# grayhong/self-diagnosing-gan

Hardware: AMD Instinct MI355X
Metric: images/sec (G+D step) (higher is better)
Workload: dtype f32

## Files before the change

### self-diagnosing-gan_amd/csrc/conv_wgrad.hip

```cpp
#include "conv_common.h"
#include "switches.h"
#include <stdlib.h>
#include <type_traits>


namespace diagan {
bool wgrad_wino_supported(int Hi, int Wi, int Ci, int Ho, int Wo, int Co, int R, int S, int sy, int dr, int off, int up,
                          int Kp);
int wgrad_wino_splits(int B, int Ho, int Wo, int Ci, int Co);
int launch_wgrad_wino(WgradArgs a, int splits, int segments, hipStream_t st);
int launch_wgrad_wino_batched(const WgradArgs* jobs, const int* splits, const int* segments, int n, hipStream_t st);
int wgrad_wino_batch_max();
bool wgrad_x3_takes(const WgradArgs& a, bool x3_on);
int launch_wgrad_x3(const WgradArgs& a, int splits, hipStream_t st);
void wgrad_x3_set(int on);


template <int BNn, int BNk, int PRO, bool P2>
__device__ __forceinline__ void conv_wgrad_body(const WgradArgs& a, const int bid, const int nblk) {
  constexpr int BK = 32;
  constexpr int TM = BNn / 64, TN = BNk / 64;
  constexpr int AC = BNn / 4, BC = BNk / 4;
  constexpr int AJ = BK * AC / 256, BJ = BK * BC / 256;
  constexpr int APR = 256 / AC, BPR = 256 / BC;
// ... 356 lines not shown
        for (int u = 0; u < U; ++u)
          t[u][r] = __builtin_bit_cast(f32x4, __builtin_amdgcn_raw_buffer_load_b128(src, voff[u] + (unsigned)r * sbytes, 0, 0));
#pragma unroll
      for (int u = 0; u < U; ++u) {
#pragma unroll
        for (int w = 1; w < R; w <<= 1)
#pragma unroll
          for (int r = 0; r + w < R; r += 2 * w) t[u][r] += t[u][r + w];
        acc[u] += t[u][0];
      }
    }
    if (sn) {
      double dot = 0.0;
      const __amdgpu_buffer_rsrc_t wsrc = __builtin_amdgcn_make_buffer_rsrc(const_cast<float*>(L.W), 0, L.n_w * 4, 0x00020000);
      const __amdgpu_buffer_rsrc_t dst = __builtin_amdgcn_make_buffer_rsrc(sl, 0, L.n_elem * 4, 0x00020000);
      f32x4 wv[U];
#pragma unroll
      for (int u = 0; u < U; ++u) wv[u] = __builtin_bit_cast(f32x4, __builtin_amdgcn_raw_buffer_load_b128(wsrc, voff[u], 0, 0));
#pragma unroll
      for (int u = 0; u < U; ++u) {
        const f32x4 g = acc[u];
        if (L.splits > 1)
          __builtin_amdgcn_raw_buffer_store_b128(__builtin_bit_cast(u32x4_t, g), dst, voff[u], 0, 0);
        dot += (double)g[0] * wv[u][0] + (double)g[1] * wv[u][1] + (double)g[2] * wv[u][2] + (double)g[3] * wv[u][3];
        acc[u] = z4;
      }
      dot = wave_sum(dot);
      __syncthreads();
      if ((threadIdx.x & 63) == 0) red[threadIdx.x >> 6] = dot;
      __syncthreads();
      if (threadIdx.x == 0) L.partials[c][lb] = (red[0] + red[1]) + (red[2] + red[3]);
    }
  }
  if (!sn) {
    const __amdgpu_buffer_rsrc_t gsrc = __builtin_amdgcn_make_buffer_rsrc(L.grad, 0, L.n_elem * 4, 0x00020000);
    f32x4 og[U];
#pragma unroll
    for (int u = 0; u < U; ++u) og[u] = __builtin_bit_cast(f32x4, __builtin_amdgcn_raw_buffer_load_b128(gsrc, voff[u], 0, 0));
#pragma unroll
    for (int u = 0; u < U; ++u)
      __builtin_amdgcn_raw_buffer_store_b128(__builtin_bit_cast(u32x4_t, og[u] + acc[u]), gsrc, voff[u], 0, 0);
  }
}

template <typename F>
__device__ __forceinline__ void fin_dispatch(int U, F&& f) {
  switch (U) {
    case 8: f(std::integral_constant<int, 8>{}); break;
    case 4: f(std::integral_constant<int, 4>{}); break;
    case 2: f(std::integral_constant<int, 2>{}); break;
    default: f(std::integral_constant<int, 1>{}); break;
  }
}

__global__ __launch_bounds__(256) __attribute__((amdgpu_waves_per_eu(4, 4))) void wgrad_finish_a_kernel(const WgFinish* __restrict__ tab, int n_layers) {
  const WgFinish L = load_uniform(tab + find_layer(tab, n_layers, blockIdx.x));
  const int lb = blockIdx.x - L.first_block;
  const int U = fin_u(L.splits);
  if ((long)lb * 1024 * U >= L.n_elem) return;
  __shared__ double red[4];
  fin_dispatch(U, [&](auto u) { fin_a<decltype(u)::value>(L, lb, red); });
}

__global__ __launch_bounds__(256) void wgrad_finish_dot_kernel(const WgFinish* __restrict__ tab) {
  const WgFinish L = tab[blockIdx.x];
  if (L.W == nullptr) return;
  __shared__ double red[256];
  const int fe = 1024 * fin_u(L.splits), nparts = (L.n_elem + fe - 1) / fe;
  for (int c = 0; c < L.nctx; ++c) {
    double d = 0.0;
    for (int k = threadIdx.x; k < nparts; k += 256) d += L.partials[c][k];
    red[threadIdx.x] = d;
    __syncthreads();
    for (int w = 128; w > 0; w >>= 1) {
      if ((int)threadIdx.x < w) red[threadIdx.x] += red[threadIdx.x + w];
      __syncthreads();
    }
    if (threadIdx.x == 0) L.partials[c][nparts] = red[0];
    __syncthreads();
  }
}

template <int U>
__device__ __forceinline__ void fin_b(const WgFinish& L, int lb) {
  constexpr int ELEMS = 1024 * U;
  constexpr int UC = U > 1 ? 2 : 1;
  const int nparts = (L.n_elem + ELEMS - 1) / ELEMS;
  float inv[2] = {0.f, 0.f}, coef[2] = {0.f, 0.f};
#pragma unroll
  for (int c = 0; c < 2; ++c) {
    if (c >= L.nctx) break;
    inv[c] = L.state[c][1];
    coef[c] = (float)(L.partials[c][nparts] * (double)inv[c]);
  }
  const int Co = L.n_w / L.Kp;
  const __amdgpu_buffer_rsrc_t gsrc = __builtin_amdgcn_make_buffer_rsrc(L.grad, 0, L.n_elem * 4, 0x00020000);
  __amdgpu_buffer_rsrc_t qsrc[2], vsrc[2], usrc[2];
#pragma unroll
  for (int c = 0; c < 2; ++c) {
    const bool on = c < L.nctx;
    qsrc[c] = __builtin_amdgcn_make_buffer_rsrc(L.slab[c], 0, on ? L.n_elem * 4 : 0, 0x00020000);
    vsrc[c] = __builtin_amdgcn_make_buffer_rsrc(const_cast<float*>(L.v[c]), 0, on ? L.Kp * 4 : 0, 0x00020000);
    usrc[c] = __builtin_amdgcn_make_buffer_rsrc(const_cast<float*>(L.u[c]), 0, on ? Co * 4 : 0, 0x00020000);
  }
#pragma unroll
  for (int u0 = 0; u0 < U; u0 += UC) {
    unsigned po[UC];
    bool okw[UC];
    f32x4 og[UC], gq[UC][2], vv[UC][2];
    float uu[UC][2];
#pragma unroll
    for (int i = 0; i < UC; ++i) {
      const long pos = (long)lb * ELEMS + ((u0 + i) * 256 + threadIdx.x) * 4;
      po[i] = pos < L.n_elem ? (unsigned)pos * 4u : 0x80000000u;
      okw[i] = pos < L.n_w;
      const unsigned n = okw[i] ? (unsigned)pos / (unsigned)L.Kp : 0u;
      const unsigned ko = okw[i] ? ((unsigned)pos - n * (unsigned)L.Kp) * 4u : 0x80000000u;
      const unsigned no = okw[i] ? n * 4u : 0x80000000u;
      og[i] = __builtin_bit_cast(f32x4, __builtin_amdgcn_raw_buffer_load_b128(gsrc, po[i], 0, 0));
#pragma unroll
      for (int c = 0; c < 2; ++c) {
        gq[i][c] = __builtin_bit_cast(f32x4, __builtin_amdgcn_raw_buffer_load_b128(qsrc[c], po[i], 0, 0));
        vv[i][c] = __builtin_bit_cast(f32x4, __builtin_amdgcn_raw_buffer_load_b128(vsrc[c], ko, 0, 0));
        uu[i][c] = __builtin_bit_cast(float, __builtin_amdgcn_raw_buffer_load_b32(usrc[c], no, 0, 0));
      }
    }
#pragma unroll
    for (int i = 0; i < UC; ++i) {
      f32x4 o = og[i];
#pragma unroll
      for (int c = 0; c < 2; ++c) {
        const f32x4 w = (gq[i][c] - (uu[i][c] * coef[c]) * vv[i][c]) * inv[c];
        o += okw[i] ? w : gq[i][c];
      }
      __builtin_amdgcn_raw_buffer_store_b128(__builtin_bit_cast(u32x4_t, o),
                                             gsrc, po[i], 0, 0);
    }
    __builtin_amdgcn_sched_barrier(0);
  }
}

__global__ __launch_bounds__(256) void wgrad_finish_b_kernel(const WgFinish* __restrict__ tab, int n_layers) {
  const WgFinish L = load_uniform(tab + find_layer(tab, n_layers, blockIdx.x));
  const int lb = blockIdx.x - L.first_block;
  const int U = fin_u(L.splits);
  if (L.W == nullptr || (long)lb * 1024 * U >= L.n_elem) return;
  fin_dispatch(U, [&](auto u) { fin_b<decltype(u)::value>(L, lb); });
}

extern "C" __attribute__((visibility("default"))) int diagan_wgrad_finish_block_elems(int splits) { return 1024 * fin_u(splits); }

}

using namespace diagan;
extern "C" int diagan_conv_gemm_get_wino(void);
extern "C" int diagan_conv_gemm_get_x3b(void);
extern "C" int diagan_conv_wgrad_splits(int M, int Co, int Kp);
extern "C" int diagan_conv_wgrad_uses_wino(int Hi, int Wi, int Ci, int Ho, int Wo, int Co, int R, int S, int sy, int dr,
                                           int off, int up, int Kp);

DIAGAN_API int diagan_wgrad_finish_batched(const void* table_dev, int n_layers, int64_t total_blocks, int any_sn,
                                           void* stream) {
  DG_REQUIRE(table_dev && n_layers > 0 && total_blocks > 0 && total_blocks < (1L << 31), "wgrad_finish_batched: bad args");
  static_assert(sizeof(WgFinish) == 128, "descriptor layout");
  const WgFinish* tab = (const WgFinish*)table_dev;
  hipStream_t st = (hipStream_t)stream;
  hipLaunchKernelGGL(wgrad_finish_a_kernel, dim3((unsigned)total_blocks), dim3(256), 0, st, tab, n_layers);
  if (any_sn) {
    hipLaunchKernelGGL(wgrad_finish_dot_kernel, dim3(n_layers), dim3(256), 0, st, tab);
    hipLaunchKernelGGL(wgrad_finish_b_kernel, dim3((unsigned)total_blocks), dim3(256), 0, st, tab, n_layers);
  }
  return check_launch("wgrad_finish_batched");
}

static void wgrad_tile(int Co, int Kp, int* bn, int* bk) {
  *bn = Co <= 64 ? 64 : 128;
  *bk = Kp <= 64 ? 64 : 128;
  if (*bn == 128 && *bk == 64) *bn = 64;
}

static void wgrad_gemm_fields(WgradArgs& a, int* bn, int* bk, bool* p2) {
  const ConvGeom& g = a.g;
  wgrad_tile(g.Co, g.Kp, bn, bk);
  a.tiles = cdiv(g.Co, *bn) * cdiv(g.Kp, *bk);
  a.same = (g.Hi == g.Ho && g.Wi == g.Wo && g.sy == 1 && g.up == 1) ? 1 : 0;
  *p2 = (g.Ho & (g.Ho - 1)) == 0 && (g.Wo & (g.Wo - 1)) == 0;
  a.lgW = a.lgHW = 0;
  while ((1 << a.lgW) < g.Wo) ++a.lgW;
  while ((1 << a.lgHW) < g.Ho * g.Wo) ++a.lgHW;
}

static int wgrad_fill_args(WgradArgs& a, const float* dy, const float* x, float* slab, int splits, int segments,
                           int64_t slab_stride, int64_t bias_off, const float* pro_scale, const float* pro_shift, int pro_mode, int B,
                           int Hi, int Wi, int Ci, int Ho, int Wo, int Co, int R, int S, int sy, int dr, int off, int up, int Kp) {
  DG_REQUIRE(dy && x && slab, "conv_wgrad: null tensor");
  DG_REQUIRE(B > 0 && Hi > 0 && Wi > 0 && Ho > 0 && Wo > 0 && R > 0 && S > 0, "conv_wgrad: bad dims");
  DG_REQUIRE(Ci > 0 && (Ci & 3) == 0 && Co > 0 && (Co & 3) == 0, "conv_wgrad: Ci=%d, Co=%d must be multiples of 4", Ci, Co);
  DG_REQUIRE(up == 1 || up == 2, "conv_wgrad: up=%d unsupported", up);
  DG_REQUIRE(dr == 1 || dr == -1, "conv_wgrad: dr must be +-1");
  DG_REQUIRE(Kp % 32 == 0 && Kp >= R * S * Ci, "conv_wgrad: bad Kp=%d", Kp);
  DG_REQUIRE(splits >= 1, "conv_wgrad: splits=%d", splits);
  DG_REQUIRE(pro_mode >= 0 && pro_mode <= PRO_BOX_RELU, "conv_wgrad: bad pro_mode %d", pro_mode);
  DG_REQUIRE(!(pro_mode == PRO_BOX || pro_mode == PRO_BOX_RELU) || (up == 1 && dr == 1 && Hi >= 2 && Wi >= 2),
             "conv_wgrad: the box-sum loader (pro_mode 5 / 6) gathers forward geometries without up-sampling");
  DG_REQUIRE(!(pro_mode == PRO_AFFINE_RELU || pro_mode == PRO_AFFINE) || (pro_scale && pro_shift),
             "conv_wgrad: affine prologue needs scale/shift");
  DG_REQUIRE(slab_stride >= (int64_t)Co * Kp && (bias_off < 0 || bias_off + Co <= slab_stride),
             "conv_wgrad: slab_stride=%ld too small for Co*Kp=%ld (+bias)", (long)slab_stride, (long)Co * Kp);
  DG_REQUIRE((long)Co * Kp * 4 < (1L << 31), "conv_wgrad: weight tensor must be smaller than 2 GiB");
  DG_REQUIRE((long)B * Ho * Wo * Co * 4 < (1L << 31) && (long)B * Hi * Wi * Ci * 4 < (1L << 31),
             "conv_wgrad: tensors must be smaller than 2 GiB (32-bit buffer offsets)");
  a.dy = dy; a.x = x; a.slab = slab; a.pro_scale = pro_scale; a.pro_shift = pro_shift; a.pro_mode = pro_mode;
  a.M = B * Ho * Wo;
  a.g = ConvGeom{B, Hi, Wi, Ci, Ho, Wo, Co, R, S, sy, dr, off, up, R * S * Ci, Kp};
  a.dWo = make_fastdiv((unsigned)Wo);
  a.dHo = make_fastdiv((unsigned)Ho);
  a.adv_b = 32 / (Ho * Wo);
  a.adv_y = (32 % (Ho * Wo)) / Wo;
  a.adv_x = (32 % (Ho * Wo)) % Wo;
  const int total_steps = cdiv(a.M, 32);
  DG_REQUIRE(segments >= 1 && splits % segments == 0, "conv_wgrad: splits=%d not a multiple of segments=%d", splits, segments);
  DG_REQUIRE(segments == 1 || (a.M % (32 * segments)) == 0, "conv_wgrad: %d pixels do not split into %d segments of whole K-steps", a.M, segments);
  a.seg_steps = cdiv(total_steps, segments);
  a.splits_per_seg = splits / segments;
  a.steps_per_split = cdiv(a.seg_steps, a.splits_per_seg);
  a.slab_stride = slab_stride;
  a.bias_off = bias_off;
  return DIAGAN_OK;
}

DIAGAN_API int diagan_conv_wgrad(const float* dy, const float* x, float* slab, int splits, int segments,
                                 int64_t slab_stride, int64_t bias_off, const float* pro_scale, const float* pro_shift, int pro_mode, int B,
                                 int Hi, int Wi, int Ci, int Ho, int Wo, int Co, int R, int S, int sy,
                                 int dr, int off, int up, int Kp, void* stream) {
  WgradArgs a;
  const int rc = wgrad_fill_args(a, dy, x, slab, splits, segments, slab_stride, bias_off, pro_scale, pro_shift, pro_mode, B, Hi, Wi, Ci,
                                 Ho, Wo, Co, R, S, sy, dr, off, up, Kp);
  if (rc != DIAGAN_OK) return rc;
  hipStream_t st = (hipStream_t)stream;
  if (diagan_conv_wgrad_uses_wino(Hi, Wi, Ci, Ho, Wo, Co, R, S, sy, dr, off, up, Kp))
    return launch_wgrad_wino(a, splits, segments, st);
  int bn, bk;
  bool p2;
  wgrad_gemm_fields(a, &bn, &bk, &p2);
  if (bn == 128 && bk == 128 && wgrad_x3_takes(a, diagan_conv_gemm_get_x3b() != 0)) return launch_wgrad_x3(a, splits, st);
  const dim3 grid(a.tiles * splits);
#define DG_WG(BN_, PRO_) do { if (p2) hipLaunchKernelGGL((conv_wgrad_kernel<BN_, 128, PRO_, true>), grid, dim3(256), 0, st, a); \
                              else hipLaunchKernelGGL((conv_wgrad_kernel<BN_, 128, PRO_, false>), grid, dim3(256), 0, st, a); } while (0)
#define DG_WG_ALL(BN_) switch (pro_mode) { \
      case PRO_NONE: DG_WG(BN_, PRO_NONE); break; \
      case PRO_RELU: DG_WG(BN_, PRO_RELU); break; \
// ... 156 lines not shown
```

### self-diagnosing-gan_amd/csrc/weight_prep.hip

```cpp
#include "conv_common.h"

namespace diagan {

__global__ __launch_bounds__(256) void sn_gemv_cols_kernel(const float* __restrict__ W, const float* __restrict__ u,
                                                           float* __restrict__ v_raw, int Co, int Kp) {
  const int k = blockIdx.x * 256 + threadIdx.x;
  if (k >= Kp) return;
  float s = 0.f;
  for (int n = 0; n < Co; ++n) s = fmaf(u[n], W[(long)n * Kp + k], s);
  v_raw[k] = s;
}

__global__ __launch_bounds__(256) void sn_gemv_rows_kernel(const float* __restrict__ W, const float* __restrict__ v_raw,
                                                           float* __restrict__ t_raw, int Co, int Kp) {
  const int n = blockIdx.x * 4 + (threadIdx.x >> 6);
  if (n >= Co) return;
  const int lane = threadIdx.x & 63;
  float s = 0.f;
  for (int k = lane * 4; k < Kp; k += 256) {
    const f32x4 w = *reinterpret_cast<const f32x4*>(W + (long)n * Kp + k);
    const f32x4 v = *reinterpret_cast<const f32x4*>(v_raw + k);
    s += w[0] * v[0] + w[1] * v[1] + w[2] * v[2] + w[3] * v[3];
  }
  s = wave_sum(s);
// ... 335 lines not shown
  }
  const float sigma = block_sum_256(s, red);
  if (threadIdx.x == 0) {
    L.state[0] = sigma;
    L.state[1] = 1.f / sigma;
    if (update_buffers) L.sigma_buf[0] = sigma;
  }
}

constexpr int PACK_MAX_LAYERS = 64;
constexpr int PACK_GRID = 2048;
__global__ __launch_bounds__(256) void pack_batched_kernel(const SnLayer* __restrict__ tab, int n_layers, int write_wd) {
  __shared__ float tile[32][33];
  __shared__ int first[PACK_MAX_LAYERS + 1];
  if (threadIdx.x == 0) {
    int acc = 0;
    for (int l = 0; l < n_layers; ++l) {
      first[l] = acc;
      const bool live = tab[l].Wf || (tab[l].Wd && write_wd);
      acc += live ? tab[l].RS * ((tab[l].Ci + 31) / 32) * ((tab[l].Co + 31) / 32) : 0;
    }
    first[n_layers] = acc;
  }
  __syncthreads();
  const int total = first[n_layers];
  const int tx = threadIdx.x & 31, ty = threadIdx.x >> 5;
  int l = 0;
  for (int item = blockIdx.x; item < total; item += gridDim.x) {
    while (first[l + 1] <= item) ++l;
    const SnLayer L = tab[l];
    const int tc = (L.Ci + 31) / 32, tn = (L.Co + 31) / 32;
    int r = item - first[l];
    const int tap = r / (tc * tn);
    r -= tap * (tc * tn);
    const int co0 = (r / tc) * 32, ci0 = (r % tc) * 32;
    const float inv = L.state[1];
    for (int q = ty; q < 32; q += 8) {
      const int co = co0 + q, ci = ci0 + tx;
      float v = 0.f;
      if (co < L.Co && ci < L.Ci) {
        v = L.W[(long)co * L.Kp + tap * L.Ci + ci] * inv;
        if (L.Wf) L.Wf[(long)co * L.Kp + tap * L.Ci + ci] = v;
      }
      tile[q][tx] = v;
    }
    __syncthreads();
    if (L.Wd && write_wd) {
      for (int q = ty; q < 32; q += 8) {
        const int ci = ci0 + q, co = co0 + tx;
        if (ci < L.Ci && co < L.Co) L.Wd[(long)ci * L.Kd + tap * L.Co + co] = tile[tx][q];
      }
    }
    __syncthreads();
  }
}

}

DIAGAN_API int diagan_sn_prepare_batched(const void* table_dev, int n_layers, int max_Co, int max_Ci, int max_RS,
                                         int max_Kp, float eps, int update_buffers, int write_wd, void* stream) {
  DG_REQUIRE(table_dev && n_layers > 0 && max_Co > 0 && max_Ci > 0 && max_RS > 0 && max_Kp > 0,
             "sn_prepare_batched: bad args");
  DG_REQUIRE(max_Kp <= SN_MAX_KP, "sn_prepare_batched: Kp=%d exceeds the LDS-resident limit %d", max_Kp, SN_MAX_KP);
  DG_REQUIRE(n_layers <= PACK_MAX_LAYERS, "sn_prepare_batched: at most %d layers per table", PACK_MAX_LAYERS);
  static_assert(sizeof(SnLayer) == 96, "descriptor layout");
  hipStream_t st = (hipStream_t)stream;
  const SnLayer* tab = (const SnLayer*)table_dev;
  hipLaunchKernelGGL(sn_cols_batched_kernel, dim3(cdiv(max_Kp, 64), SN_RSPLIT, n_layers), dim3(256), 0, st, tab);
  hipLaunchKernelGGL(sn_rows_batched_kernel, dim3(cdiv(max_Co, 8), 1, n_layers), dim3(256), 0, st, tab);
  hipLaunchKernelGGL(sn_finalize_batched_kernel, dim3(1, 1, n_layers), dim3(256), 0, st, tab, eps, update_buffers);
  if (write_wd >= 0)
    hipLaunchKernelGGL(pack_batched_kernel, dim3(PACK_GRID), dim3(256), 0, st, tab, n_layers, write_wd);
  return check_launch("sn_prepare_batched");
}

DIAGAN_API int diagan_pack_batched(const void* table_dev, int n_layers, int max_Co, int max_Ci, int max_RS,
                                   int write_wd, void* stream) {
  DG_REQUIRE(table_dev && n_layers > 0 && max_Co > 0 && max_Ci > 0 && max_RS > 0, "pack_batched: bad args");
  DG_REQUIRE(n_layers <= PACK_MAX_LAYERS, "pack_batched: at most %d layers per table", PACK_MAX_LAYERS);
  hipLaunchKernelGGL(pack_batched_kernel, dim3(PACK_GRID), dim3(256), 0, (hipStream_t)stream, (const SnLayer*)table_dev,
                     n_layers, write_wd);
  return check_launch("pack_batched");
}
```

### self-diagnosing-gan_amd/diagan/models/layers.py

```python

import os

import torch
import torch.nn as nn

from diagan.ops import conv as C
from diagan.ops import eltwise as E

WGRAD_BOX = os.environ.get("DIAGAN_WGRAD_BOX", "1") != "0"


def _r4(n):
    return (n + 3) // 4 * 4


class ConvLayer(nn.Module):

    def __init__(self, kind, in_ch, out_ch, ksize, stride=1, pad=0, bias=True, sn=False, xavier_gain=None):
        super().__init__()
        self.kind, self.in_ch, self.out_ch, self.ksize = kind, in_ch, out_ch, ksize
        self.Cip, self.Cop = _r4(in_ch), _r4(out_ch)
        self.geom = C.Geom(kind, self.Cip, self.Cop, ksize, ksize, stride, pad)
        self.sn = sn
        ref = (nn.Conv2d if kind == 'conv' else nn.ConvTranspose2d)(in_ch, out_ch, ksize, stride, pad, bias=bias)
        self._oihw_shape = tuple(ref.weight.shape)
        self.weight = nn.Parameter(self._pack(ref.weight.data))
        if bias:
            b = torch.zeros(self.Cop)
            b[:out_ch] = ref.bias.data
            self.bias = nn.Parameter(b)
        else:
            self.bias = None
        if sn:
            self.register_buffer('sn_u', torch.randn(1, out_ch))
            self.register_buffer('sn_sigma', torch.ones(1))
        self._wd = None
        self._wd_version = -1
        self._register_state_dict_hook(self._sd_hook)
        self._register_load_state_dict_pre_hook(self._load_hook)
        if xavier_gain is not None:
            self.xavier_(xavier_gain)

    def xavier_(self, gain):
        w = torch.empty(self._oihw_shape)
        nn.init.xavier_uniform_(w, gain)
        self.weight.data.copy_(self._pack(w).to(self.weight.device))
        return self

    def _pack(self, w):
        if self.kind == 'convT':
            w = w.permute(1, 0, 2, 3)
        Co, Ci, R, S = w.shape
        wp = w.permute(0, 2, 3, 1)
        wp = torch.nn.functional.pad(wp, (0, self.Cip - Ci))
        out = torch.zeros((self.Cop, self.geom.Kp), dtype=w.dtype, device=w.device)
        out[:Co, : R * S * self.Cip] = wp.reshape(Co, -1)
        return out

    def _unpack(self, wp):
        R = self.ksize
        w = wp[: self.out_ch, : R * R * self.Cip].reshape(self.out_ch, R, R, self.Cip)[..., : self.in_ch]
        w = w.permute(0, 3, 1, 2)
        if self.kind == 'convT':
            w = w.permute(1, 0, 2, 3)
        return w.contiguous()

    @staticmethod
    def _sd_hook(module, sd, prefix, local_metadata):
        sd[prefix + 'weight'] = module._unpack(sd[prefix + 'weight'])
        if module.bias is not None:
            sd[prefix + 'bias'] = sd[prefix + 'bias'][: module.out_ch].clone()
        return sd

    def _load_hook(self, sd, prefix, *args):
        k = prefix + 'weight'
        if k in sd and sd[k].dim() == 4:
            sd[k] = self._pack(sd[k].to(torch.float32))
        k = prefix + 'bias'
        if k in sd and sd[k].numel() == self.out_ch and self.out_ch != self.Cop:
            b = torch.zeros(self.Cop, dtype=torch.float32, device=sd[k].device)
            b[: self.out_ch] = sd[k]
            sd[k] = b
        net = getattr(self, '_net', None)
        if net is not None:
            net.param_version += 1

    class Ctx:
        __slots__ = ("wf", "wd", "u", "v", "state", "_keep", "row_scale", "pair", "wkey", "wver")

        def __init__(self):
            self.row_scale = None
            self.pair = None
# ... 322 lines not shown
            p0, p1 = ctx.pair
            gx, _, _ = E.head_bwd(dlogit, self.weight.data, p0.state[1:], ctx.x, ctx.pooled, need_gx=True,
                                  need_wgrad=False, inv_sigma1=p1.state[1:])
            if need_wgrad:
                h = dlogit.numel() // 2
                for p, sl in ((p0, slice(0, h)), (p1, slice(h, 2 * h))):
                    _, G, dot = E.head_bwd(dlogit[sl], self.weight.data, None, ctx.x[sl], ctx.pooled[sl], need_gx=False,
                                           need_wgrad=True, dbias=self.bias.grad)
                    nat.call("diagan_sn_grad_fix", nat.ptr(G), nat.ptr(dot), 1, nat.ptr(p.u), nat.ptr(p.v),
                             nat.ptr(p.state), nat.ptr(self.weight.grad), 1, self.in_ch, 1, nat.current_stream())
            return gx
        inv = ctx.state[1:] if self.sn else None
        gx, G, dot = E.head_bwd(dlogit, self.weight.data, inv, ctx.x, ctx.pooled, need_gx=True,
                                need_wgrad=need_wgrad, dbias=self.bias.grad if need_wgrad else None)
        if need_wgrad:
            if self.sn:
                from diagan import _native as nat
                nat.call("diagan_sn_grad_fix", nat.ptr(G), nat.ptr(dot), 1, nat.ptr(ctx.u), nat.ptr(ctx.v),
                         nat.ptr(ctx.state), nat.ptr(self.weight.grad), 1, self.in_ch, 1, nat.current_stream())
            else:
                E.add(self.weight.grad.view(-1), G, out=self.weight.grad.view(-1))
        return gx


class SNBatch:

    def __init__(self, net, layers, n_slots=2):
        import numpy as np
        from diagan import _native as nat
        self.net, self.layers, self.nat = net, layers, nat
        dev = net.flat_params.device
        self.slab_generation = net.slab_generation
        desc = np.dtype([('p', np.uint64, 9), ('i', np.int32, 6)])
        self.tables = []
        f32 = dict(dtype=torch.float32, device=dev)
        dims = []
        for slot in range(n_slots):
            tab = np.zeros(len(layers), dtype=desc)
            for li, m in enumerate(layers):
                if isinstance(m, ConvLayer):
                    g = m.geom
                    Co, Ci, RS, Kp, Kd = g.Co, g.Ci, g.R * g.S, g.Kp, g.Kd
                    wf, wd = torch.zeros((Co, Kp), **f32), torch.zeros((Ci, Kd), **f32)
                    ctx = ConvLayer.Ctx()
                else:
                    Co, Ci, RS, Kp, Kd = 1, m.in_ch, 1, m.in_ch, 0
                    wf = wd = None
                    ctx = HeadLinear.Ctx()
                ctx.u, ctx.v, ctx.state = torch.zeros(Co, **f32), torch.zeros(Kp, **f32), torch.ones(2, **f32)
                if isinstance(m, ConvLayer):
                    ctx.wf, ctx.wd, ctx.wkey = wf, wd, slot
                work = torch.zeros(8 * Kp + Co, **f32)
                ctx._keep = (work,)
                if not hasattr(m, '_slot_ctx') or m._slot_ctx is None or len(m._slot_ctx) != n_slots:
                    m._slot_ctx = [None] * n_slots
                m._slot_ctx[slot] = ctx
                ptrs = [m.weight.data.data_ptr(), m.sn_u.data_ptr(), m.sn_sigma.data_ptr(), ctx.u.data_ptr(),
                        ctx.v.data_ptr(), ctx.state.data_ptr(), work.data_ptr(),
                        wf.data_ptr() if wf is not None else 0, wd.data_ptr() if wd is not None else 0]
                tab[li]['p'] = ptrs
                tab[li]['i'] = [Co, Ci, RS, Kp, Kd, 0]
                dims.append((Co, Ci, RS, Kp))
            self.tables.append(torch.from_numpy(tab.view(np.uint8).copy()).to(dev))
        self.max = [max(d[k] for d in dims) for k in range(4)]
        convs = [m for m in layers if isinstance(m, ConvLayer)]
        self.unit = torch.ones(2, **f32)
        ptab = np.zeros(len(convs), dtype=desc)
        for li, m in enumerate(convs):
            g = m.geom
            wd_raw = torch.zeros((g.Ci, g.Kd), **f32)
            pc = ConvLayer.Ctx()
            pc.wf, pc.wd = m.weight.data, wd_raw
            pc.u = pc.v = pc.state = None
            pc.row_scale = (m._slot_ctx[0].state[1:], m._slot_ctx[1].state[1:])
            pc.pair = (m._slot_ctx[0], m._slot_ctx[1])
            pc.wkey = 'pair'
            m._pair_ctx = pc
            ptab[li]['p'] = [m.weight.data.data_ptr(), 0, 0, 0, 0, self.unit.data_ptr(), 0, 0, wd_raw.data_ptr()]
            ptab[li]['i'] = [g.Co, g.Ci, g.R * g.S, g.Kp, g.Kd, 0]
        self.pair_table = torch.from_numpy(ptab.view(np.uint8).copy()).to(dev)
        self.n_convs = len(convs)
        self.pair_version = None
        self.convs = convs
        self.runs = 0
        self.slot_ver = {}

    def stale(self):
        self.net.flat_params
        return self.slab_generation != self.net.slab_generation

    def run_pair(self, training, need_dgrad):
        self.run(0, training, -1)
        self.run(1, training, -1)
        if need_dgrad and self.pair_version != self.net.param_version:
            nat = self.nat
            nat.call("diagan_pack_batched", self.pair_table.data_ptr(), self.n_convs, self.max[0], self.max[1],
                     self.max[2], 1, nat.current_stream())
            self.pair_version = self.net.param_version
        for m in self.convs:
            m._pair_ctx.wver = ('p', self.net.param_version)

    def run(self, slot, training, write_wd):
        nat = self.nat
        nat.call("diagan_sn_prepare_batched", self.tables[slot].data_ptr(), len(self.layers), self.max[0],
                 self.max[1], self.max[2], self.max[3], 1e-12, 1 if training else 0,
                 write_wd if isinstance(write_wd, int) and not isinstance(write_wd, bool) else (1 if write_wd else 0),
                 nat.current_stream())
        if write_wd != -1:
            self.runs += 1
            self.slot_ver[slot] = ('s', self.runs)
            for m in self.convs:
                m._slot_ctx[slot].wver = self.slot_ver[slot]


class WgradEntry:
    __slots__ = ("owner", "slot", "M", "n_w", "n_elem", "stride", "splits", "own_splits", "bias_off", "segments", "slab",
                 "partials", "sn_ctx")

    def __init__(self, owner, slot, M, n_w, stride, splits, bias_off, segments, dev):
        self.owner, self.slot, self.M, self.n_w, self.n_elem, self.stride = owner, slot, M, n_w, stride, stride
        self.splits, self.own_splits, self.bias_off, self.segments, self.sn_ctx = splits, splits, bias_off, segments, None
        self.slab = torch.empty(splits * stride, dtype=torch.float32, device=dev)
        self.partials = torch.empty((segments, (stride + 1023) // 1024 + 1), dtype=torch.float64, device=dev)

    def set_splits(self, splits):
        if splits != self.splits:
            self.splits = splits
            self.slab = torch.empty(splits * self.stride, dtype=torch.float32, device=self.slab.device)
            self.owner.drop_tables(self.slot)


class WgradBatch:
    QUEUE_BYTES = int(os.environ.get("DIAGAN_WGRAD_QUEUE_BYTES", str(8 << 30)))

    def __init__(self, net):
        self.net = net
        self.entries = {}
        self.launched = {}
        self.tables = {}
        self.slab_generation = None
        self.hold = False
        self.pending = []
        self.overlapped = 0
        self.queue = {}
        self.queued_bytes = {}
        self.batch_plans = {}
        self.job_tables = {}
        self.batched_launches = 0

    def drop_tables(self, slot):
        self.tables = {k: v for k, v in self.tables.items() if k[0] != slot}

    def _entry(self, layer, slot, M, segments, dy_shape, x_shape, geom):
        self.net.flat_grads
        if self.slab_generation != self.net.slab_generation:
            self.entries.clear(), self.tables.clear(), self.job_tables.clear()
            self.slab_generation = self.net.slab_generation
        e = self.entries.get((layer, slot))
        if e is None or e.M != M:
            g = geom if geom is not None else layer.geom
            n_w = g.Co * g.Kp
            has_bias = layer.bias is not None
            n_b = layer.bias.numel() if has_bias else 0
            if has_bias and layer.bias.grad.data_ptr() != layer.weight.grad.data_ptr() + 4 * n_w:
                raise RuntimeError("bias gradient does not follow the weight gradient in the flat slab")
            stride = n_w + n_b
            base = C.wgrad_splits_geom(g, dy_shape[0], x_shape[1], x_shape[2], dy_shape[1], dy_shape[2])
            splits = max(segments, base // segments * segments)
            if segments == 1 and C.small_co_wgrad(g):
                splits = C.small_co_wgrad_splits(dy_shape[0], dy_shape[1])
            e = self.entries[(layer, slot)] = WgradEntry(self, slot, M, n_w, stride, splits, n_w if has_bias else -1, segments,
                                                         layer.weight.device)
            self.drop_tables(slot)
        return e

    def launch(self, layer, slot, dy, x, pro, sn_ctx, segments=1, geom=None):
        M = dy.numel() // dy.shape[-1]
        if self.hold and slot in self.pending:
            self.pending.remove(slot)
            self.flush(slot)
            self._finish_layers(slot, self.launched.pop(slot, []))
        xs = C.wg_x_shape(x, pro)
        e = self._entry(layer, slot, M, segments, tuple(dy.shape), xs, geom)
        e.sn_ctx = sn_ctx
        self.launched.setdefault(slot, []).append(layer)
        g, pooled = (geom, True) if geom is not None else (layer.geom, False)
        if C.WGRAD_BATCH and dy.dim() == 4 and x.dim() == 4:
            mode = int(pro[0]) if pro is not None else 0
            if not (segments == 1 and C.small_co_wgrad(g)) and C.wgrad_batch_class(g, xs[1], xs[2], dy.shape[1], dy.shape[2], mode):
                shape = C.WgradShape(g, tuple(dy.shape), tuple(xs), mode, segments, e.own_splits, pooled)
                self.queue.setdefault(slot, []).append(C.WgradJob(layer, dy, x, pro, e, shape))
                self.queued_bytes[slot] = self.queued_bytes.get(slot, 0) + 4 * (dy.numel() + x.numel())
                if self.queued_bytes[slot] > self.QUEUE_BYTES:
                    self.flush(slot)
                return
        C.conv_wgrad_into(g, dy, x, e.slab, e.splits, e.stride, e.bias_off, pro=pro, segments=segments, pooled=pooled)

    def flush(self, slot):
        jobs = self.queue.pop(slot, None)
        self.queued_bytes.pop(slot, None)
        if not jobs:
            return
        key = tuple(j.shape for j in jobs)
        plan = self.batch_plans.get(key)
        if plan is None:
            plan = self.batch_plans[key] = C.wgrad_launch_plan(key)
        for n, launch in enumerate(plan):
            part = [jobs[j] for j in launch.jobs]
            for job, splits in zip(part, launch.splits):
                job.entry.set_splits(splits)
            if len(part) > 1:
                C.conv_wgrad_batched(part, launch.kernel_name, flop_scale=4.0 if launch.pooled else 1.0, key=(key, n),
                                     cache=self.job_tables)
                self.batched_launches += 1
            else:
                job, e = part[0], part[0].entry
                C.conv_wgrad_into(job.shape.geom, job.dy, job.x, e.slab, e.splits, e.stride, e.bias_off, pro=job.pro,
                                  segments=job.shape.segments, pooled=launch.pooled)

    def finish(self, slot):
        self.flush(slot)
        if self.hold:
            self.pending.append(slot)
            return
        self._finish_layers(slot, self.launched.pop(slot, []))

    def split_for_overlap(self, slot):
        layers = self.launched.get(slot, [])
        if len(layers) < 2:
            return None
        base = self.net.flat_grads.data_ptr()
        lo = [(l.weight.grad.data_ptr() - base) // 4 for l in layers]
        hi = [o + self.entries[(l, slot)].n_elem for o, l in zip(lo, layers)]
        total, acc, best = sum(b - a for a, b in zip(lo, hi)), 0, None
        for h in range(1, len(layers)):
            acc += hi[h - 1] - lo[h - 1]
            cut = min(lo[:h])
            if cut % 4 == 0 and all(b <= cut for b in hi[h:]):
                score = abs(2 * acc - total)
                if best is None or score < best[0]:
                    best = (score, h, cut)
        if best is None:
            return None
        _, h, cut = best
        return layers[:h], layers[h:], cut

    def _finish_layers(self, slot, layers):
        import numpy as np
        from diagan import _native as nat
        if not layers:
            return
        key = (slot, tuple(id(l) for l in layers))
        t = self.tables.get(key)
        if t is None:
            desc = np.dtype([('p', np.uint64, 12), ('stride', np.int64), ('i', np.int32, 6)])
            tab = np.zeros(len(layers), dtype=desc)
            any_sn, total_blocks = 0, 0
            for li, layer in enumerate(layers):
                e = self.entries[(layer, slot)]
                c = e.sn_ctx
                ctxs = list(c) if isinstance(c, tuple) else [c]
                nctx = len(ctxs)
                per = e.splits // nctx
                sn = ctxs[0] is not None
                any_sn |= int(sn)
                pp = [0] * 12
                for pi, cc in enumerate(ctxs):
                    pp[0 + pi] = e.slab.data_ptr() + 4 * pi * per * e.stride
                    if sn:
                        pp[2 + pi], pp[4 + pi], pp[6 + pi] = cc.u.data_ptr(), cc.v.data_ptr(), cc.state.data_ptr()
                    pp[8 + pi] = e.partials[pi].data_ptr()
                if not sn and nctx > 1:
                    nctx, per = 1, e.splits
                pp[10] = layer.weight.grad.data_ptr()
                pp[11] = layer.weight.data.data_ptr() if sn else 0
                assert 64 * e.stride < 2 ** 31, "wgrad finish: 16 splits of a layer must fit a 2 GiB buffer window"
                tab[li]['p'], tab[li]['stride'] = pp, e.stride
                tab[li]['i'] = [per, e.n_elem, e.n_w, layer.geom.Kp, nctx, total_blocks]
                be = nat.fn("diagan_wgrad_finish_block_elems")(per)
                total_blocks += (e.n_elem + be - 1) // be
            t = (torch.from_numpy(tab.view(np.uint8).copy()).to(layers[0].weight.device), len(layers), total_blocks, any_sn)
            self.tables[key] = t
        nat.call("diagan_wgrad_finish_batched", t[0].data_ptr(), t[1], t[2], t[3], nat.current_stream())


class FlatNet(nn.Module):

    def __init__(self):
        super().__init__()
        self.param_version = 0
        self.slab_generation = 0
        self._flat = None
        self._flat_grad = None
        object.__setattr__(self, 'wgrad_batch', WgradBatch(self))
        object.__setattr__(self, '_wino_batches', {})

    def wino_batch(self, key):
        b = self._wino_batches.get(key)
        if b is None:
            b = self._wino_batches[key] = C.WinoWeightBatch()
        return b

    def _link_layers(self):
        for m in self.modules():
            if m is not self:
                object.__setattr__(m, '_net', self)

    def __deepcopy__(self, memo):
        import copy
        new = self.__class__.__new__(self.__class__)
        memo[id(self)] = new
        for k, v in self.__dict__.items():
            if k == 'wgrad_batch':
                continue
            new.__dict__[k] = {} if k == '_wino_batches' else (None if k in ('_flat', '_flat_grad') else copy.deepcopy(v, memo))
        new.__dict__['wgrad_batch'] = WgradBatch(new)
        for m in new.modules():
            if isinstance(m, ConvLayer):
                m.__dict__.pop('_wsites', None)
                m._wd = None
        if self._flat is not None:
            new._build_flat()
        new.slab_generation = self.slab_generation + 1
        return new

    def _build_flat(self):
        params = list(self.parameters())
        if not params:
            return
        dev = params[0].device
        total = sum(_r4(p.numel()) for p in params)
        flat = torch.zeros(total, dtype=torch.float32, device=dev)
        grad = torch.zeros(total, dtype=torch.float32, device=dev)
        off = 0
        for p in params:
            n = p.numel()
            flat[off: off + n].copy_(p.data.reshape(-1))
            p.data = flat[off: off + n].view(p.shape)
            p.grad = grad[off: off + n].view(p.shape)
            off += _r4(n)
        self._flat, self._flat_grad = flat, grad
        self.param_version += 1
        self.slab_generation += 1

    def _apply(self, fn, recurse=True):
        out = super()._apply(fn)
        self._build_flat()
        self._wino_batches.clear()
        for m in self.modules():
            if isinstance(m, ConvLayer):
                m._wd = None
                m.__dict__.pop('_wsites', None)
        return out

    def zero_grad(self, set_to_none=False):
        if self._flat_grad is None:
            self._build_flat()
        self._flat_grad.zero_()
        self.wgrad_batch.hold, self.wgrad_batch.pending = False, []
        self.wgrad_batch.queue.clear()
        self.wgrad_batch.queued_bytes.clear()

    @property
# ... 77 lines not shown
```

Baseline: 5354.

## Fuse paired spectral-norm power iterations and fold wgrad dot into finish kernel

Adds a sn_pair_kernel that runs the spectral-norm power iteration for both slots and the optional stale weight pack in fewer launches. It keeps small weight tiles in LDS and passes partial norms through a scratch buffer. Separately, the wgrad finish path gets a bdot kernel where every block redundantly reduces the per-layer partial dot products, removing the single-grid dot kernel launch when the part count is small. This trades redundant reductions and extra LDS use for fewer kernel launches and serialization points.

```diff
diff --git a/include/diagan_sn_pair.h b/include/diagan_sn_pair.h
--- /dev/null
+++ b/include/diagan_sn_pair.h
@@ -0,0 +1,19 @@
+#ifndef DIAGAN_SN_PAIR_H
+#define DIAGAN_SN_PAIR_H
+
+#include <stdint.h>
+
+#ifdef __cplusplus
+extern "C" {
+#endif
+
+int64_t diagan_sn_pair_scratch_floats(int n_layers, int max_Co, int max_Kp);
+
+int diagan_sn_prepare_pair(const void* slot0_table_dev, const void* slot1_table_dev, int n_layers, const void* pair_table_dev,
+                           int n_pair, int max_Co, int max_Kp, float* scratch, int64_t scratch_floats, float eps,
+                           int update_buffers, int pack_stale, void* stream);
+
+#ifdef __cplusplus
+}
+#endif
+#endif
diff --git a/self-diagnosing-gan_amd/csrc/conv_wgrad.hip b/self-diagnosing-gan_amd/csrc/conv_wgrad.hip
--- a/self-diagnosing-gan_amd/csrc/conv_wgrad.hip
+++ b/self-diagnosing-gan_amd/csrc/conv_wgrad.hip
@@ -462,7 +462,7 @@
 }
 
 template <int U>
-__device__ __forceinline__ void fin_b(const WgFinish& L, int lb) {
+__device__ __forceinline__ void fin_b(const WgFinish& L, int lb, const double* dots = nullptr, const float* invs = nullptr) {
   constexpr int ELEMS = 1024 * U;
   constexpr int UC = U > 1 ? 2 : 1;
   const int nparts = (L.n_elem + ELEMS - 1) / ELEMS;
@@ -470,8 +470,8 @@
 #pragma unroll
   for (int c = 0; c < 2; ++c) {
     if (c >= L.nctx) break;
-    inv[c] = L.state[c][1];
-    coef[c] = (float)(L.partials[c][nparts] * (double)inv[c]);
+    inv[c] = invs ? invs[c] : L.state[c][1];
+    coef[c] = (float)((dots ? dots[c] : L.partials[c][nparts]) * (double)inv[c]);
   }
   const int Co = L.n_w / L.Kp;
   const __amdgpu_buffer_rsrc_t gsrc = __builtin_amdgcn_make_buffer_rsrc(L.grad, 0, L.n_elem * 4, 0x00020000);
@@ -528,6 +528,41 @@
   fin_dispatch(U, [&](auto u) { fin_b<decltype(u)::value>(L, lb); });
 }
 
+__global__ __launch_bounds__(256) void wgrad_finish_bdot_kernel(const WgFinish* __restrict__ tab, int n_layers) {
+  const WgFinish L = load_uniform(tab + find_layer(tab, n_layers, blockIdx.x));
+  const int lb = blockIdx.x - L.first_block;
+  const int U = fin_u(L.splits);
+  if (L.W == nullptr || (long)lb * 1024 * U >= L.n_elem) return;
+  __shared__ double red[2][256];
+  __shared__ double dots[2];
+  const int fe = 1024 * U, nparts = (L.n_elem + fe - 1) / fe;
+  float invs[2] = {0.f, 0.f};
+#pragma unroll
+  for (int c = 0; c < 2; ++c) {
+    double d = 0.0;
+    if (c < L.nctx) {
+      invs[c] = L.state[c][1];
+      for (int k = threadIdx.x; k < nparts; k += 256) d += L.partials[c][k];
+    }
+    red[c][threadIdx.x] = d;
+  }
+  __syncthreads();
+  for (int w = 128; w > 0; w >>= 1) {
+    if ((int)threadIdx.x < w) {
+      red[0][threadIdx.x] += red[0][threadIdx.x + w];
+      red[1][threadIdx.x] += red[1][threadIdx.x + w];
+    }
+    __syncthreads();
+  }
+  if (threadIdx.x < 2 && (int)threadIdx.x < L.nctx) {
+    const double d = red[threadIdx.x][0];
+    dots[threadIdx.x] = d;
+    if (lb == 0) (threadIdx.x ? L.partials[1] : L.partials[0])[nparts] = d;
+  }
+  __syncthreads();
+  fin_dispatch(U, [&](auto u) { fin_b<decltype(u)::value>(L, lb, dots, invs); });
+}
+
 extern "C" __attribute__((visibility("default"))) int diagan_wgrad_finish_block_elems(int splits) { return 1024 * fin_u(splits); }
 
 }
@@ -546,7 +581,9 @@
   const WgFinish* tab = (const WgFinish*)table_dev;
   hipStream_t st = (hipStream_t)stream;
   hipLaunchKernelGGL(wgrad_finish_a_kernel, dim3((unsigned)total_blocks), dim3(256), 0, st, tab, n_layers);
-  if (any_sn) {
+  if (any_sn == 2) {
+    hipLaunchKernelGGL(wgrad_finish_bdot_kernel, dim3((unsigned)total_blocks), dim3(256), 0, st, tab, n_layers);
+  } else if (any_sn) {
     hipLaunchKernelGGL(wgrad_finish_dot_kernel, dim3(n_layers), dim3(256), 0, st, tab);
     hipLaunchKernelGGL(wgrad_finish_b_kernel, dim3((unsigned)total_blocks), dim3(256), 0, st, tab, n_layers);
   }
diff --git a/self-diagnosing-gan_amd/csrc/weight_prep.hip b/self-diagnosing-gan_amd/csrc/weight_prep.hip
--- a/self-diagnosing-gan_amd/csrc/weight_prep.hip
+++ b/self-diagnosing-gan_amd/csrc/weight_prep.hip
@@ -441,3 +441,236 @@
                      n_layers, write_wd);
   return check_launch("pack_batched");
 }
+
+namespace diagan {
+
+constexpr int SNP_LDS_ROWS = 128;
+constexpr int SNP_LD = 65;
+constexpr int SNP_MAX_CO = 1024;
+constexpr int SNP_MAX_SLICES = 256;
+
+struct SnPairArgs {
+  const SnLayer* prev;
+  const SnLayer* dup;
+  const SnLayer* cur;
+  const SnLayer* pack;
+  float* scratch;
+  int n_pack, max_Co, max_slices, prev_half, cur_half, write_bufs;
+  float eps;
+};
+
+__global__ __launch_bounds__(256) void sn_pair_kernel(const SnPairArgs a) {
+  __shared__ float ws[SNP_LDS_ROWS * SNP_LD];
+  __shared__ float part[SN_RSPLIT][4][64];
+  __shared__ float us[SNP_MAX_CO];
+  __shared__ float nvs[SNP_MAX_SLICES];
+  __shared__ float vs[64];
+  __shared__ float red[4];
+  __shared__ int pidx;
+  const int tid = threadIdx.x;
+  const SnLayer L = (a.cur ? a.cur : a.prev)[blockIdx.z];
+  const int k0 = blockIdx.x * 64;
+  const int slices = (L.Kp + 63) / 64;
+  if (k0 >= L.Kp || L.Co > a.max_Co || slices > a.max_slices) return;
+  const long half = (long)a.max_slices * (a.max_Co + 1);
+  float* lay = a.scratch + (long)blockIdx.z * 2 * half;
+  const int Co = L.Co, Kp = L.Kp;
+  const bool in_lds = Co <= SNP_LDS_ROWS;
+  const f32x4 z4 = {0.f, 0.f, 0.f, 0.f};
+
+  f32x4 w4[SNP_LDS_ROWS / 16];
+  const int c4 = (tid & 15) * 4, r0 = tid >> 4;
+  if (a.cur && in_lds) {
+#pragma unroll
+    for (int i = 0; i < SNP_LDS_ROWS / 16; ++i) {
+      const int n = r0 + 16 * i;
+      w4[i] = (n < Co && k0 + c4 < Kp) ? *reinterpret_cast<const f32x4*>(L.W + (long)n * Kp + k0 + c4) : z4;
+    }
+  }
+  const float* mine = (a.pack && tid < a.n_pack) ? a.pack[tid].W : nullptr;
+  if (tid == 0) pidx = 0x7fffffff;
+
+  if (a.prev) {
+    const SnLayer P = a.prev[blockIdx.z];
+    const float* nvp = lay + a.prev_half * half;
+    const float* tp = nvp + a.max_slices;
+    const float v_prev = (tid < 64 && k0 + tid < Kp) ? P.v_out[k0 + tid] : 0.f;
+    const int tot = Co * slices;
+    const bool staged = tot <= SNP_LDS_ROWS * SNP_LD;
+    if (tid < slices) nvs[tid] = nvp[tid];
+    if (staged) {
+#pragma unroll 16
+      for (int e = tid; e < tot; e += 256) ws[e] = tp[e];
+    }
+    __syncthreads();
+    float nv2 = 0.f;
+    for (int s = 0; s < slices; ++s) nv2 += nvs[s];
+    const float nv = fmaxf(sqrtf(nv2), a.eps);
+    float s2 = 0.f;
+    for (int n = tid; n < Co; n += 256) {
+      float t = 0.f;
+      if (staged) {
+#pragma unroll 4
+        for (int s = 0; s < slices; ++s) t += ws[s * Co + n];
+      } else {
+#pragma unroll 8
+        for (int s = 0; s < slices; ++s) t += tp[(long)s * Co + n];
+      }
+      t = t / nv;
+      us[n] = t;
+      s2 += t * t;
+    }
+    const float nt = fmaxf(sqrtf(block_sum_256(s2, red)), a.eps);
+    float s3 = 0.f;
+    for (int n = tid; n < Co; n += 256) {
+      const float t = us[n];
+      const float un = t / nt;
+      us[n] = un;
+      s3 += un * t;
+    }
+    const float sigma = block_sum_256(s3, red);
+    if (tid < 64 && k0 + tid < Kp) {
+      const float v = v_prev / nv;
+      P.v_out[k0 + tid] = v;
+      if (a.dup) a.dup[blockIdx.z].v_out[k0 + tid] = v;
+    }
+    if (blockIdx.x == 0) {
+      for (int c = 0; c < 2; ++c) {
+        if (c == 1 && !a.dup) break;
+        const SnLayer O = c ? a.dup[blockIdx.z] : P;
+        for (int n = tid; n < Co; n += 256) O.u_out[n] = us[n];
+        if (tid == 0) {
+          O.state[0] = sigma;
+          O.state[1] = 1.f / sigma;
+        }
+      }
+      if (a.write_bufs) {
+        for (int n = tid; n < Co; n += 256) P.u_buf[n] = us[n];
+        if (tid == 0) P.sigma_buf[0] = sigma;
+      }
+    }
+  }
+  if (!a.cur) return;
+
+  if (!a.prev)
+    for (int n = tid; n < Co; n += 256) us[n] = L.u_buf[n];
+  if (in_lds) {
+#pragma unroll
+    for (int i = 0; i < SNP_LDS_ROWS / 16; ++i) {
+      const int n = r0 + 16 * i;
+      if (n < Co) {
+#pragma unroll
+        for (int j = 0; j < 4; ++j) ws[n * SNP_LD + c4 + j] = w4[i][j];
+      }
+    }
+  }
+  __syncthreads();
+  if (mine != nullptr && mine == L.W) atomicMin(&pidx, tid);
+
+  const int kl = tid & 63, rl = tid >> 6, k = k0 + kl;
+  const int per = (Co + SN_RSPLIT - 1) / SN_RSPLIT;
+#pragma unroll
+  for (int r = 0; r < SN_RSPLIT; ++r) {
+    const int n0 = r * per, n1 = min(n0 + per, Co);
+    float s = 0.f;
+    if (k < Kp) {
+      if (in_lds) {
+#pragma unroll 4
+        for (int n = n0 + rl; n < n1; n += 4) s = fmaf(us[n], ws[n * SNP_LD + kl], s);
+      } else {
+#pragma unroll 4
+        for (int n = n0 + rl; n < n1; n += 4) s = fmaf(us[n], L.W[(long)n * Kp + k], s);
+      }
+    }
+    part[r][rl][kl] = s;
+  }
+  __syncthreads();
+  const bool packing = a.pack != nullptr && pidx != 0x7fffffff;
+  SnLayer Q = L;
+  float inv = 1.f;
+  if (packing) {
+    Q = a.pack[pidx];
+    if (Q.Wd != nullptr) inv = Q.state[1];
+  }
+  const SnLayer C = a.cur[blockIdx.z];
+  float* nvp = lay + a.cur_half * half;
+  float* tp = nvp + a.max_slices;
+  if (rl == 0) {
+    float v = 0.f;
+#pragma unroll
+    for (int r = 0; r < SN_RSPLIT; ++r) v += (part[r][0][kl] + part[r][1][kl]) + (part[r][2][kl] + part[r][3][kl]);
+    vs[kl] = v;
+    if (k < Kp) C.v_out[k] = v;
+    const float q = wave_sum(v * v);
+    if (kl == 0) nvp[blockIdx.x] = q;
+  }
+  __syncthreads();
+
+  const int kmax = min(64, Kp - k0);
+  for (int n = tid; n < Co; n += 256) {
+    float s = 0.f;
+    if (in_lds) {
+#pragma unroll 16
+      for (int kk = 0; kk < kmax; ++kk) s = fmaf(ws[n * SNP_LD + kk], vs[kk], s);
+    } else {
+#pragma unroll 4
+      for (int kk = 0; kk < kmax; kk += 4) {
+        const f32x4 w = *reinterpret_cast<const f32x4*>(L.W + (long)n * Kp + k0 + kk);
+#pragma unroll
+        for (int j = 0; j < 4; ++j) s = fmaf(w[j], vs[kk + j], s);
+      }
+    }
+    tp[(long)blockIdx.x * Co + n] = s;
+  }
+
+  if (packing && Q.Wd != nullptr && Q.Co == Co && Q.Kp == Kp) {
+    const int live = Q.RS * Q.Ci, lane = tid & 63;
+    for (int kk = __builtin_amdgcn_readfirstlane(tid >> 6); kk < kmax; kk += 4) {
+      const int kq = k0 + kk;
+      if (kq >= live) break;
+      const int tap = kq / Q.Ci, ci = kq - tap * Q.Ci;
+      float* dst = Q.Wd + (long)ci * Q.Kd + tap * Co;
+      for (int co = lane; co < Co; co += 64) dst[co] = (in_lds ? ws[co * SNP_LD + kk] : L.W[(long)co * Kp + kq]) * inv;
+    }
+  }
+}
+
+}
+
+DIAGAN_API int64_t diagan_sn_pair_scratch_floats(int n_layers, int max_Co, int max_Kp) {
+  if (n_layers <= 0 || max_Co <= 0 || max_Kp <= 0) return 0;
+  return (int64_t)n_layers * 2 * cdiv(max_Kp, 64) * ((int64_t)max_Co + 1);
+}
+
+DIAGAN_API int diagan_sn_prepare_pair(const void* slot0_table_dev, const void* slot1_table_dev, int n_layers,
+                                      const void* pair_table_dev, int n_pair, int max_Co, int max_Kp, float* scratch,
+                                      int64_t scratch_floats, float eps, int update_buffers, int pack_stale, void* stream) {
+  DG_REQUIRE(slot0_table_dev && slot1_table_dev && scratch && n_layers > 0 && max_Co > 0 && max_Kp > 0, "sn_prepare_pair: bad args");
+  DG_REQUIRE(n_layers <= PACK_MAX_LAYERS, "sn_prepare_pair: at most %d layers per table", PACK_MAX_LAYERS);
+  DG_REQUIRE(max_Co <= SNP_MAX_CO, "sn_prepare_pair: Co=%d exceeds the LDS-resident limit %d", max_Co, SNP_MAX_CO);
+  DG_REQUIRE(max_Kp <= 64 * SNP_MAX_SLICES, "sn_prepare_pair: Kp=%d exceeds the limit %d", max_Kp, 64 * SNP_MAX_SLICES);
+  DG_REQUIRE(!pack_stale || (pair_table_dev && n_pair > 0 && n_pair <= PACK_MAX_LAYERS),
+             "sn_prepare_pair: a stale pair operand needs a pair table of 1..%d layers", PACK_MAX_LAYERS);
+  const int64_t need = diagan_sn_pair_scratch_floats(n_layers, max_Co, max_Kp);
+  DG_REQUIRE(scratch_floats >= need, "sn_prepare_pair: scratch of %ld floats, %ld needed", (long)scratch_floats, (long)need);
+  hipStream_t st = (hipStream_t)stream;
+  const SnLayer* t0 = (const SnLayer*)slot0_table_dev;
+  const SnLayer* t1 = (const SnLayer*)slot1_table_dev;
+  SnPairArgs a;
+  a.scratch = scratch; a.max_Co = max_Co; a.max_slices = cdiv(max_Kp, 64); a.eps = eps;
+  a.pack = pack_stale ? (const SnLayer*)pair_table_dev : nullptr; a.n_pack = pack_stale ? n_pair : 0;
+  const dim3 grid(a.max_slices, 1, n_layers);
+  a.prev = nullptr; a.dup = nullptr; a.cur = t0; a.prev_half = 0; a.cur_half = 0; a.write_bufs = 0;
+  hipLaunchKernelGGL(sn_pair_kernel, grid, dim3(256), 0, st, a);
+  a.pack = nullptr; a.n_pack = 0;
+  if (update_buffers) {
+    a.prev = t0; a.cur = t1; a.prev_half = 0; a.cur_half = 1;
+    hipLaunchKernelGGL(sn_pair_kernel, grid, dim3(256), 0, st, a);
+    a.prev = t1; a.cur = nullptr; a.prev_half = 1; a.write_bufs = 1;
+    hipLaunchKernelGGL(sn_pair_kernel, grid, dim3(256), 0, st, a);
+  } else {
+    a.prev = t0; a.dup = t1; a.cur = nullptr;
+    hipLaunchKernelGGL(sn_pair_kernel, grid, dim3(256), 0, st, a);
+  }
+  return check_launch("sn_prepare_pair");
+}
diff --git a/self-diagnosing-gan_amd/diagan/_native/sn_pair_abi.py b/self-diagnosing-gan_amd/diagan/_native/sn_pair_abi.py
--- /dev/null
+++ b/self-diagnosing-gan_amd/diagan/_native/sn_pair_abi.py
@@ -0,0 +1,35 @@
+import os
+
+from diagan import _native as nat
+from diagan._native import parse_header
+
+HEADER_PATH = os.path.join(os.path.dirname(nat.HEADER_PATH), "diagan_sn_pair.h")
+
+_sigs = None
+_bound = {}
+
+
+def signatures():
+    global _sigs
+    if _sigs is None:
+        if not os.path.exists(HEADER_PATH):
+            raise RuntimeError(f"diagan_sn_pair.h not found at {HEADER_PATH}: the ctypes signatures are read from it "
+                               "(the package runs from a checkout of the repository).")
+        with open(HEADER_PATH) as f:
+            _sigs = parse_header(f.read())
+    return _sigs
+
+
+def fn(name):
+    f = _bound.get(name)
+    if f is None:
+        f = getattr(nat.lib(), name)
+        f.restype, f.argtypes = signatures()[name]
+        _bound[name] = f
+    return f
+
+
+def call(name, *args):
+    rc = fn(name)(*args)
+    if rc != 0:
+        raise RuntimeError(f"{name} failed ({rc}): {nat.last_error()}")
diff --git a/self-diagnosing-gan_amd/diagan/models/layers.py b/self-diagnosing-gan_amd/diagan/models/layers.py
--- a/self-diagnosing-gan_amd/diagan/models/layers.py
+++ b/self-diagnosing-gan_amd/diagan/models/layers.py
@@ -8,6 +8,10 @@
 from diagan.ops import eltwise as E
 
 WGRAD_BOX = os.environ.get("DIAGAN_WGRAD_BOX", "1") != "0"
+SN_PAIR = os.environ.get("DIAGAN_SN_PAIR", "1") != "0"
+SN_PAIR_MAX_CO = 128
+WGRAD_FOLD_DOT = os.environ.get("DIAGAN_WGRAD_FOLD_DOT", "1") != "0"
+WGRAD_FOLD_DOT_MAX_PARTS = 256
 
 
 def _r4(n):
@@ -496,6 +500,11 @@
         self.n_convs = len(convs)
         self.pair_version = None
         self.convs = convs
+        self.pair_fused = SN_PAIR and self.max[0] <= SN_PAIR_MAX_CO and n_slots == 2
+        if self.pair_fused:
+            from diagan._native import sn_pair_abi as snat
+            self.snat = snat
+            self.pair_scratch = torch.empty(snat.fn("diagan_sn_pair_scratch_floats")(len(layers), self.max[0], self.max[3]), **f32)
         self.runs = 0
         self.slot_ver = {}
 
@@ -504,10 +513,19 @@
         return self.slab_generation != self.net.slab_generation
 
     def run_pair(self, training, need_dgrad):
-        self.run(0, training, -1)
-        self.run(1, training, -1)
-        if need_dgrad and self.pair_version != self.net.param_version:
-            nat = self.nat
+        nat = self.nat
+        stale = need_dgrad and self.pair_version != self.net.param_version
+        if self.pair_fused:
+            self.snat.call("diagan_sn_prepare_pair", self.tables[0].data_ptr(), self.tables[1].data_ptr(), len(self.layers),
+                           self.pair_table.data_ptr(), self.n_convs, self.max[0], self.max[3], self.pair_scratch.data_ptr(),
+                           self.pair_scratch.numel(), 1e-12, 1 if training else 0, 1 if stale else 0, nat.current_stream())
+            if stale:
+                self.pair_version = self.net.param_version
+            stale = False
+        else:
+            self.run(0, training, -1)
+            self.run(1, training, -1)
+        if stale:
             nat.call("diagan_pack_batched", self.pair_table.data_ptr(), self.n_convs, self.max[0], self.max[1],
                      self.max[2], 1, nat.current_stream())
             self.pair_version = self.net.param_version
@@ -669,7 +687,7 @@
         if t is None:
             desc = np.dtype([('p', np.uint64, 12), ('stride', np.int64), ('i', np.int32, 6)])
             tab = np.zeros(len(layers), dtype=desc)
-            any_sn, total_blocks = 0, 0
+            any_sn, total_blocks, most_parts = 0, 0, 0
             for li, layer in enumerate(layers):
                 e = self.entries[(layer, slot)]
                 c = e.sn_ctx
@@ -693,6 +711,10 @@
                 tab[li]['i'] = [per, e.n_elem, e.n_w, layer.geom.Kp, nctx, total_blocks]
                 be = nat.fn("diagan_wgrad_finish_block_elems")(per)
                 total_blocks += (e.n_elem + be - 1) // be
+                if sn:
+                    most_parts = max(most_parts, (e.n_elem + be - 1) // be)
+            if any_sn and WGRAD_FOLD_DOT and most_parts <= WGRAD_FOLD_DOT_MAX_PARTS:
+                any_sn = 2
             t = (torch.from_numpy(tab.view(np.uint8).copy()).to(layers[0].weight.device), len(layers), total_blocks, any_sn)
             self.tables[key] = t
         nat.call("diagan_wgrad_finish_batched", t[0].data_ptr(), t[1], t[2], t[3], nat.current_stream())
```

Result: no change. 5382, median of 6 (+0.5%).
